# aleju/face-generator

Hardware: NVIDIA H100
Metric: 32x32 GAN train images/sec (1 D-iter + 1 G-iter per batch, batch 256/GPU) (higher is better)
Workload: dtype f32

## Files before the change

face_generator_b200/csrc/capi.cu:

```cuda
#include <algorithm>
#include <cstdarg>
#include <cstdlib>
#include <cstring>

#include "fg_internal.h"
#include "k_conv_tc.h"

static thread_local char g_err[1024] = "";
void fg_set_error(const char* fmt, ...) {
  va_list ap;
  va_start(ap, fmt);
  vsnprintf(g_err, sizeof(g_err), fmt, ap);
  va_end(ap);
}

#define ENTER(c)                                      \
  do {                                                \
    if (!(c)) {                                       \
      fg_set_error("null fg_ctx");                    \
      return FG_ERR_INVALID;                          \
    }                                                 \
    FG_CUDA(cudaSetDevice((c)->device));              \
  } while (0)

// ... 48 lines not shown
  auto dalloc = [c](auto** p, size_t n) { return fg_dalloc(c, c->allocs, reinterpret_cast<float**>(p), n); };
  FG_TRY(dalloc(&c->lop_sx, 2));
  FG_TRY(dalloc(&c->lop_sy, 2));
  FG_TRY(dalloc(&c->seed_dev, 2 * kMaxIters));
  c->splitk_ws_elems = (size_t)c->sm_count * 4 * 128 * 128;
  FG_TRY(dalloc(&c->splitk_ws, c->splitk_ws_elems));
  c->red_ws_elems = (size_t)4 << 20;
  FG_TRY(dalloc(&c->red_ws, 2 * c->red_ws_elems));
  FG_TRY(dalloc(&c->red_ws_opt, 2 * kOptRedRows));
  FG_TRY(dalloc(&c->red_ticket, 2));
  FG_TRY(dalloc(&c->bwd_claim, 1));
  FG_TRY(dalloc(&c->small_ws, (size_t)kSmallMaxParts * 9 * 4 * 128));
  FG_TRY(dalloc(&c->bn_acc, 4 * 256 * 2));
  FG_TRY(dalloc(&c->bn_slice_acc, 32 * 4 * 256 * 2 + 64));
  FG_TRY(dalloc(&c->bn_parts, B * 3072));
  c->io_dev_elems = std::max<size_t>(B * 1024 * C, B * kMaskPerSample);
  return dalloc(&c->io_dev, c->io_dev_elems);
}
void ctx_free(fg_ctx* c) {
  for (void* p : c->allocs) cudaFree(p);
  c->allocs.clear();
  for (int i = 0; i < 8; ++i)
    if (c->scratch[i]) cudaFree(c->scratch[i]);
}
}

extern "C" {

const char* fg_version(void) { return "fg_b200 0.1 (sm_90a)"; }
const char* fg_last_error(void) { return g_err; }
// ... 44 lines not shown
  if (r != FG_OK) {
    net32_free(c);
    ctx_free(c);
    cudaStreamDestroy(c->stream);
    delete c;
    return r;
  }
  *out = c;
  return FG_OK;
}

int fg_destroy(fg_ctx* c) {
  if (!c) return FG_OK;
  cudaSetDevice(c->device);
  cudaStreamSynchronize(c->stream);
  if (c->comm_stream) {
    cudaStreamSynchronize(c->comm_stream);
    cudaStreamDestroy(c->comm_stream);
    cudaEventDestroy(c->ev_fork);
    cudaEventDestroy(c->ev_join);
  }
  tc_destroy(c);
  net32_free(c);
  ctx_free(c);
  for (auto& kv : c->timers)
    for (auto& pr : kv.second.pending) {
      cudaEventDestroy(pr.first);
      cudaEventDestroy(pr.second);
    }
  if (c->own_stream && c->stream) cudaStreamDestroy(c->stream);
  delete c;
  return FG_OK;
}

int fg_set_stream(fg_ctx* c, void* s) {
  ENTER(c);
// ... 213 lines not shown
```

face_generator_b200/csrc/convl.cu:

```cuda
#include "convl.h"

#include "k_conv_tc.h"
#include "k_misc.h"

int convl_dalloc(ConvLEnv& e, float** p, size_t elems) { return fg_dalloc(e.c, *e.allocs, p, elems); }

int ScalePairs::alloc(fg_ctx* c, std::vector<void*>& allocs, int pairs) {
  n = pairs;
  used = 0;
  return fg_dalloc(c, allocs, &base, 2 * (size_t)pairs);
}
int ScalePairs::take(float** pair) {
  if (used == n) {
    fg_set_error("a block of %d FP16 scale pairs is full", n);
    return FG_ERR_UNSUPPORTED;
  }
  *pair = base + 2 * used++;
  return FG_OK;
}
int ScalePairs::reset(fg_ctx* c) const {
  if (!tc_f16(c)) return FG_OK;
  FG_CUDA(cudaMemset2DAsync(base, 2 * sizeof(float), 0, sizeof(float), n, c->stream));
  return FG_OK;
}
// ... 13 lines not shown
      op.split_ready = false;
      return FG_OK;
    }
    return tc_split(c, x, op.hi, op.lo, n);
  }
  if (op.amax_ready) op.amax_ready = false;
  else FG_TRY(tc_amax(c, x, n, op.s));
  return tc_split_h(c, x, op.hi, op.lo, n, op.s);
}

int convl_alloc(ConvLEnv& e, ConvL& L) {
  const size_t nw = (size_t)L.k * L.k * L.Cout * L.Cin;
  FG_TRY(convl_dalloc(e, &L.Wp, nw));
  FG_TRY(convl_dalloc(e, &L.Wpd, nw));
  if (L.nA) FG_TRY(convl_dalloc(e, &L.bp, L.Cout));
  if (!L.x.s) FG_TRY(convl_dalloc(e, &L.x.s, 2));
  if (!e.dy.s) FG_TRY(convl_dalloc(e, &e.dy.s, 2));
  if (tc_conv_eligible(L.geom_k(e.maxB))) {
    const int K = L.geom_k(e.maxB).Cin;
    const size_t nk = (size_t)L.k * L.k * L.Cout * K, nx = (size_t)e.maxB * L.H * L.H * K;
    FG_TRY(convl_dalloc(e, &L.Wf_hi, nk));
    FG_TRY(convl_dalloc(e, &L.Wf_lo, nk));
    FG_TRY(convl_dalloc(e, &L.x.hi, nx));
    FG_TRY(convl_dalloc(e, &L.x.lo, nx));
    if (L.kpad) {
      FG_TRY(convl_dalloc(e, &L.Wpad, nk));
      FG_TRY(convl_dalloc(e, &L.xpad, nx));
    }
  }
  if (L.need_dgrad && tc_conv_eligible(L.geom_d(e.maxB))) {
    FG_TRY(convl_dalloc(e, &L.Wd_hi, nw));
    FG_TRY(convl_dalloc(e, &L.Wd_lo, nw));
  }
  const int B = e.maxB;
  if (L.pad_out && !(tc_conv_eligible(ConvGeom{B, L.H, L.H, L.Cin, L.pad_out, L.k, 1}) &&
                     tc_conv_eligible(ConvGeom{B, L.H, L.H, L.pad_out, L.Cin, L.k, 1}) && L.Cin % 128 == 0))
    L.pad_out = 0;
  if (L.pad_dy && !(L.x.hi && tc_conv_eligible(ConvGeom{B, L.H, L.H, L.Cin, L.pad_dy, L.k, 1}) && L.Cin % 64 == 0))
    L.pad_dy = 0;
  if (L.pad_out) {
    const size_t nq = (size_t)L.k * L.k * L.pad_out * L.Cin;
    FG_TRY(convl_dalloc(e, &L.Wq_hi, nq));
    FG_TRY(convl_dalloc(e, &L.Wq_lo, nq));
    const size_t nx = (size_t)B * L.H * L.H * L.Cin;
    FG_TRY(convl_dalloc(e, &L.x.hi, nx));
    FG_TRY(convl_dalloc(e, &L.x.lo, nx));
  }
  return FG_OK;
}

int convl_pack(fg_ctx* c, ConvL& L, const float* P) {
  const int KK = L.k * L.k;
  const bool tc_on = c->conv_impl != FG_CONV_SIMT;
  const bool h = tc_on && tc_f16(c) && L.geom_k(1).Cin % 64 == 0 && (L.Cout % 64 == 0 || L.pad_out);
  L.packed_f16 = h;
  if (KK > 1 && tc_on && !L.nA && !L.cA && !L.pad_out && !L.kpad && L.Wf_hi && (L.Wd_hi || !L.need_dgrad) && tc_f(c, L, 1) &&
      (!L.need_dgrad || tc_d(c, L, 1))) {
    if (h) return tc_pack_split_h(c, P + L.w_off, L.Wf_hi, L.Wf_lo, L.Wd_hi, L.Wd_lo, L.Cout, L.Cin, KK);
    return tc_pack_split(c, P + L.w_off, L.Wf_hi, L.Wf_lo, L.Wd_hi, L.Wd_lo, L.Cout, L.Cin, KK);
  }
  FG_TRY(k_pack_weights(c, P + L.w_off, L.Wp, L.need_dgrad ? L.Wpd : nullptr, L.Cout, L.Cin, KK, L.nA, L.nS, L.cA, L.cS));
  if (L.bp) FG_TRY(k_pack_weights(c, P + L.b_off, L.bp, nullptr, L.Cout, 1, 1, L.nA, L.nS, 0, 0));
// ... 107 lines not shown

bool upsl_tc(const fg_ctx* c, const UpsL& U) {
  return c->conv_impl != FG_CONV_SIMT && tc_conv_eligible(U.geom(1)) && U.Cout % 128 == 0 && U.Cin % 64 == 0;
}

int upsl_alloc(ConvLEnv& e, UpsL& U) {
  const size_t nw25 = (size_t)25 * U.Cout * U.Cin, nw36 = (size_t)36 * U.Cout * U.Cin;
  FG_TRY(convl_dalloc(e, &U.Wp, nw25));
  FG_TRY(convl_dalloc(e, &U.Wpd, nw25));
  FG_TRY(convl_dalloc(e, &U.Wf_hi, nw36));
  FG_TRY(convl_dalloc(e, &U.Wf_lo, nw36));
  FG_TRY(convl_dalloc(e, &U.Wd_hi, nw36));
  FG_TRY(convl_dalloc(e, &U.Wd_lo, nw36));
  FG_TRY(convl_dalloc(e, &U.Wx_hi, nw25));
  FG_TRY(convl_dalloc(e, &U.Wx_lo, nw25));
  const size_t nx = (size_t)e.maxB * (U.H / 2) * (U.H / 2) * U.Cin;
  FG_TRY(convl_dalloc(e, &U.x.hi, nx));
  FG_TRY(convl_dalloc(e, &U.x.lo, nx));
  if (!U.x.s) FG_TRY(convl_dalloc(e, &U.x.s, 2));
  return FG_OK;
}

int upsl_pack(fg_ctx* c, UpsL& U, const float* P) {
  const float* W = P + U.w_off;
  if (!upsl_tc(c, U)) return k_pack_weights(c, W, U.Wp, U.Wpd, U.Cout, U.Cin, 25, 0, 0, 0, 0);
  if (tc_f16(c)) FG_TRY(tc_pack_collapsed_h(c, W, U.Wf_hi, U.Wf_lo, U.Wd_hi, U.Wd_lo, U.Cout, U.Cin));
  else FG_TRY(tc_pack_collapsed(c, W, U.Wf_hi, U.Wf_lo, U.Wd_hi, U.Wd_lo, U.Cout, U.Cin));
  if (c->conv_impl == FG_CONV_TC_DENSE) FG_TRY(tc_pack_split(c, W, U.Wx_hi, U.Wx_lo, nullptr, nullptr, U.Cout, U.Cin, 25));
  return FG_OK;
}
// ... 53 lines not shown
```

face_generator_b200/csrc/convl.h:

```cpp
#pragma once
#include <vector>

#include "fg_internal.h"

inline bool tc_f16(const fg_ctx* c) { return c->mma_f16 && c->conv_impl == FG_CONV_TC_COLLAPSED; }

struct AmaxInto {
  fg_ctx* c;
  AmaxInto(fg_ctx* c_, TcOp& op) : AmaxInto(c_, op.s, &op.amax_ready) {}
  AmaxInto(fg_ctx* c_, float* pair, bool* done) : c(c_) {
    if (tc_f16(c)) {
      c->amax_out = reinterpret_cast<unsigned*>(pair);
      c->amax_done = done;
    }
  }
  ~AmaxInto() { c->amax_out = nullptr; }
};

inline unsigned* take_amax(fg_ctx* c) {
  unsigned* p = c->amax_out;
  if (p) *c->amax_done = true;
  return p;
}

int tc_op_split(fg_ctx* c, TcOp& op, const float* x, int64_t n, bool f16);

inline int pack_key(const fg_ctx* c) { return c->conv_impl | (c->mma_f16 << 4); }
int convl_dalloc(ConvLEnv& e, float** p, size_t elems);
int convl_alloc(ConvLEnv& e, ConvL& L);
bool convl_tc_fwd(const fg_ctx* c, const ConvL& L);
bool convl_tc_bwd(const fg_ctx* c, const ConvL& L);
int convl_pack(fg_ctx* c, ConvL& L, const float* P);
int convl_fwd(ConvLEnv& e, ConvL& L, const float* in, const float* P, float* out, int B);
int convl_bwd(ConvLEnv& e, ConvL& L, const float* in, const float* dy, float* G, float* din, int B);

bool upsl_tc(const fg_ctx* c, const UpsL& U);
int upsl_alloc(ConvLEnv& e, UpsL& U);
int upsl_pack(fg_ctx* c, UpsL& U, const float* P);
int upsl_fwd(ConvLEnv& e, UpsL& U, const float* h, const float* P, float* z, int B, int* parts = nullptr);
int upsl_bwd(ConvLEnv& e, UpsL& U, TcOp& dy, const float* h, const float* dz, float* G, float* dh, int B, bool* pooled);

int gen_alloc(ConvLEnv& e, UpsGen& G, const GenDesc& d);
int gen_pack(fg_ctx* c, UpsGen& G, NetPair& p);
int gen_forward(ConvLEnv& e, UpsGen& G, NetPair& p, const float* noise, int B, bool training);
int gen_backward(ConvLEnv& e, UpsGen& G, NetPair& p, const float* dy, float* dnoise);
void gen_debug_rows(const UpsGen& G, std::vector<DebugTensor>& rows);
```

face_generator_b200/csrc/fg_internal.h:

```cpp
#pragma once
#include <cuda_runtime.h>
#include <cstdint>
#include <cstdio>
#include <deque>
#include <functional>
#include <initializer_list>
#include <map>
#include <string>
#include <vector>

#include "fg_b200.h"

void fg_set_error(const char* fmt, ...);

#define FG_CUDA(call)                                                                               \
  do {                                                                                              \
    cudaError_t e__ = (call);                                                                       \
    if (e__ != cudaSuccess) {                                                                       \
      fg_set_error("%s:%d: %s -> %s", __FILE__, __LINE__, #call, cudaGetErrorString(e__));          \
      return FG_ERR_CUDA;                                                                           \
    }                                                                                               \
  } while (0)
#define FG_TRY(call)                  \
  do {                                \
// ... 143 lines not shown
};

struct UpsGen {
  int S = 32, C = 3;
  GLayout gl;
  ConvL GL1, GC3;
  UpsL GU[2];
  ScalePairs pairs;
  float* sdz[2] = {nullptr, nullptr};
  float *noise = nullptr, *z0 = nullptr, *h0 = nullptr, *z1 = nullptr, *h1 = nullptr, *z2 = nullptr, *h2 = nullptr,
        *z3 = nullptr, *y = nullptr;
  float *dz3 = nullptr, *dfull = nullptr, *dz2 = nullptr, *dz1 = nullptr, *dz0 = nullptr;
  float *bn_mean[2] = {nullptr, nullptr}, *bn_istd[2] = {nullptr, nullptr}, *bn_mg = nullptr;
  int B = 0;
  bool train = true, valid = false;
  std::deque<std::string> names;
  const char *t_bn2_finalize = nullptr, *t_bn2_stats = nullptr, *t_bn2_apply = nullptr, *t_bn2_bwd_reduce = nullptr,
             *t_bn2_bwd_apply = nullptr;
};

struct TimerRec {
  double ms = 0;
  int64_t launches = 0;
  std::vector<std::pair<cudaEvent_t, cudaEvent_t>> pending;
};

struct IterStage {
  float* p[8] = {};
  size_t cap[8] = {};
  int reserve(fg_ctx* c, std::vector<void*>& allocs, int k, size_t n);
// ... 33 lines not shown
  float* io_dev = nullptr;
  size_t io_dev_elems = 0;
  float* scratch[8] = {nullptr, nullptr, nullptr, nullptr, nullptr, nullptr, nullptr, nullptr};
  size_t scratch_elems[8] = {0, 0, 0, 0, 0, 0, 0, 0};
  void* nccl_comm = nullptr;
  int world = 1, rank = 0;
  int dp_overlap = 1;
  int reserve_sms = 0;
  int last_conv_kind = 0, last_conv_tile_m = 0, last_conv_tile_n = 0, last_conv_format = 0, last_conv_splits = 0;
  int bwd_merge = 1, bwd_merge_ctas = 0;
  int* bwd_claim = nullptr;
  int use_graph = 1, graph_epoch = 0;
  uint64_t* seed_dev = nullptr;
  cudaStream_t comm_stream = nullptr;
  cudaEvent_t ev_fork = nullptr, ev_join = nullptr;
  bool debug_keep = false;
  cudaEvent_t events[16] = {};
  bool timing = false;
  std::map<std::string, TimerRec> timers;
};

inline void note_conv(fg_ctx* c, int kind, int tile_m, int tile_n, int format, int splits) {
  c->last_conv_kind = kind;
  c->last_conv_tile_m = tile_m;
  c->last_conv_tile_n = tile_n;
  c->last_conv_format = format;
  c->last_conv_splits = splits;
}

struct ScopedTimer {
// ... 134 lines not shown
int step_check(fg_ctx* c, const char* what, int B, int nd, int ng, bool inputs, const fg_dataset* d = nullptr, bool fed = false);
struct StepNets {
  StepNets(fg_ctx* c, NetPair& pair, const fg_hyper* h, int B, float* logit, float* out, float* dlogit, float* masks,
           int64_t mask, bool gate, bool overlap)
      : c(c), pair(&pair), h(h), B(B), logit(logit), out(out), dlogit(dlogit), masks(masks), mask(mask), gate(gate),
        overlap(overlap) {}
  fg_ctx* c;
  NetPair* pair;
  const fg_hyper* h;
  int B;
  float *logit, *out, *dlogit;
  float* masks;
  int64_t mask;
  bool gate;
  bool overlap;
  virtual int g_forward(int j, bool d_iter) = 0;
  virtual int d_input(int j) = 0;
  virtual int draw_masks(int kind, const uint64_t* root) = 0;
  virtual int d_forward(bool on_g) = 0;
  virtual int d_backward(bool want_wgrad, bool want_dx) = 0;
  virtual int g_backward() = 0;
};
int pair_train_step(StepNets& s, int nd, int ng, const float* masksD, const float* masksG, uint64_t seed,
                    std::initializer_list<const void*> inputs, const std::function<int()>* feed, fg_step_stats* stats);
struct DebugTensor;
void pair_keep_rows(const NetPair& p, std::vector<DebugTensor>& ents);

int k_relu_fwd(fg_ctx* c, const float* z, float* h, int64_t n);
int k_relu_bwd(fg_ctx* c, const float* dh, const float* z, float* dz, int64_t n);
int k_tanh_dropout_fwd(fg_ctx* c, const float* z, const float* masks_in, const uint64_t* seed_dev, float p, float* code, float* h,
                       float* flags_out, int64_t n);
int k_tanh_dropout_bwd(fg_ctx* c, const float* dh, const float* masks, float p, const float* code, float* dz, int64_t n);
int k_abs_criterion(fg_ctx* c, bool sigmoid, const float* z, const float* t, float* y, float* dz, int64_t n, float* loss);

bool fg_is_dev(const void* p);
int fg_to_dev(fg_ctx* c, const float* p, size_t n, float* staging, const float** out);
int fg_to_user(fg_ctx* c, float* dst, const float* src_dev, size_t n);
// ... 29 lines not shown
```

face_generator_b200/csrc/gen.cu:

```cuda
#include "convl.h"

GLayout make_g_layout(int C, int side) {
  const int64_t n0 = 128 * (side / 4) * (side / 4);
  GLayout L;
  int64_t o = 0;
  L.L1W = o; o += n0 * kNoiseDim;
  L.L1b = o; o += n0;
  L.a1 = o; o += 1;
  L.C1W = o; o += 256 * 128 * 25;
  L.C1b = o; o += 256;
  L.g1 = o; o += 256;
  L.be1 = o; o += 256;
  L.a2 = o; o += 1;
  L.C2W = o; o += 128 * 256 * 25;
  L.C2b = o; o += 128;
  L.g2 = o; o += 128;
  L.be2 = o; o += 128;
  L.a3 = o; o += 1;
  L.C3W = o; o += (int64_t)C * 128 * 9;
  L.C3b = o; o += C;
  L.total = o;
  return L;
}

int gen_alloc(ConvLEnv& e, UpsGen& G, const GenDesc& d) {
  fg_ctx* c = e.c;
  const int S = d.side, C = c->C;
  G.S = S;
  G.C = C;
  G.gl = make_g_layout(C, S);
  const GLayout& gl = G.gl;
  auto timer = [&](const char* name) {
    G.names.push_back(std::string(d.prefix) + name);
    return G.names.back().c_str();
  };
  FG_TRY(G.pairs.alloc(c, *e.allocs, 8));
  ConvL& L1 = G.GL1;
// ... 20 lines not shown
  for (int i = 0; i < 2; ++i) {
    UpsL& U = G.GU[i];
    U.Cin = ci[i]; U.Cout = co[i]; U.H = hs[i];
    U.w_off = wo[i]; U.b_off = bo[i];
    U.tf = timer(uf[i]); U.td = timer(ud[i]); U.tw = timer(uw[i]);
    U.tb = d.bwd_merge ? timer(ub[i]) : nullptr;
    FG_TRY(G.pairs.take(&U.x.s));
    FG_TRY(G.pairs.take(&G.sdz[i]));
    FG_TRY(upsl_alloc(e, U));
  }
  G.t_bn2_finalize = timer("G.bn2.finalize");
  G.t_bn2_stats = timer("hbm.G.bn2.stats");
  G.t_bn2_apply = timer("hbm.G.bn2.apply");
  G.t_bn2_bwd_reduce = timer("hbm.G.bn2.bwd_reduce");
  G.t_bn2_bwd_apply = timer("hbm.G.bn2.bwd_apply");
  const size_t B = e.maxB, n0 = L1.Cout, n1 = (size_t)256 * (S / 2) * (S / 2), n2 = (size_t)128 * S * S, n3 = (size_t)C * S * S;
  for (auto [p, n] : {std::pair<float**, size_t>{&G.noise, kNoiseDim}, {&G.z0, n0}, {&G.h0, n0}, {&G.z1, n1}, {&G.h1, n1},
                      {&G.z2, n2}, {&G.h2, n2}, {&G.z3, n3}, {&G.y, n3}, {&G.dz3, n3},
                      {&G.dfull, (size_t)256 * S * S},
                      {&G.dz2, n2}, {&G.dz1, n1}, {&G.dz0, n0}})
    FG_TRY(convl_dalloc(e, p, B * n));
  for (int i = 0; i < 2; ++i) {
    FG_TRY(convl_dalloc(e, &G.bn_mean[i], co[i]));
    FG_TRY(convl_dalloc(e, &G.bn_istd[i], co[i]));
  }
  return convl_dalloc(e, &G.bn_mg, 512);
}

int gen_pack(fg_ctx* c, UpsGen& G, NetPair& p) {
  if (p.G_pack == pack_key(c)) return FG_OK;
  FG_TRY(convl_pack(c, G.GL1, p.PG));
  for (int i = 0; i < 2; ++i) FG_TRY(upsl_pack(c, G.GU[i], p.PG));
  FG_TRY(convl_pack(c, G.GC3, p.PG));
  p.G_pack = pack_key(c);
  return FG_OK;
}

namespace {
int bn_stats(fg_ctx* c, UpsGen& G, NetPair& p, int i, const float* z, int B, bool training, int parts, const char* t_finalize,
             const char* t_stats) {
  const int Cc = G.GU[i].Cout;
// ... 3 lines not shown
  if (parts) {
    ScopedTimer tm(c, t_finalize);
    return k_bn_finalize_parts(c, c->bn_parts, parts, 4, G.bn_mean[i], G.bn_istd[i], rm, rv, P, Cc);
  }
  {
    ScopedTimer tm(c, t_stats);
    FG_TRY(k_bn_stats(c, z, c->bn_acc, P, Cc));
  }
  return k_bn_finalize(c, c->bn_acc, G.bn_mean[i], G.bn_istd[i], rm, rv, P, Cc);
}
}

int gen_forward(ConvLEnv& e, UpsGen& G, NetPair& p, const float* noise, int B, bool training) {
  fg_ctx* c = e.c;
  FG_REQUIRE(B >= 1 && B <= e.maxB, "G forward: batch %d out of range [1,%d]", B, e.maxB);
  FG_TRY(gen_pack(c, G, p));
  const GLayout& L = G.gl;
  const float* P = p.PG;
  const int S = G.S;
  if (noise != G.noise)
    FG_CUDA(cudaMemcpyAsync(G.noise, noise, sizeof(float) * B * kNoiseDim, cudaMemcpyDeviceToDevice, c->stream));
  G.B = B;
  G.train = training;
  FG_TRY(G.pairs.reset(c));
  FG_TRY(convl_fwd(e, G.GL1, G.noise, P, G.z0, B));
  {
    AmaxInto am(c, G.GU[0].x);
    FG_TRY(k_prelu_fwd(c, G.z0, P + L.a1, G.h0, (int64_t)B * G.GL1.Cout));
  }
  int parts = training ? 1 : 0;
  FG_TRY(upsl_fwd(e, G.GU[0], G.h0, P, G.z1, B, &parts));
// ... 83 lines not shown
```

face_generator_b200/csrc/netpair.cu:

```cuda
#include <algorithm>
#include <cstdlib>
#include <cstring>

#include "convl.h"
#include "fg_internal.h"

namespace {
struct Half {
  float *P, *g, *tail, *m, *v;
  int64_t n;
};
Half half(const NetPair& p, int net) {
  if (net == FG_NET_D) return Half{p.PD, p.gD, p.tailD, p.mD, p.vD, p.nD};
  return Half{p.PG, p.gG, p.tailG, p.mG, p.vG, p.nG};
}
int* step_count(DeviceStats* s, int net) { return net == FG_NET_D ? &s->t_D : &s->t_G; }
}

int fg_dalloc(fg_ctx* c, std::vector<void*>& allocs, float** p, size_t n) {
  void* q = nullptr;
  FG_CUDA(cudaMalloc(&q, std::max<size_t>(n, 1) * sizeof(float)));
  FG_CUDA(cudaMemsetAsync(q, 0, std::max<size_t>(n, 1) * sizeof(float), c->stream));
  allocs.push_back(q);
  *p = (float*)q;
  return FG_OK;
}

int pair_alloc(fg_ctx* c, std::vector<void*>& allocs, NetPair& p, int64_t nG, int64_t nD, bool bn) {
  p.nG = nG;
  p.nD = nD;
  FG_TRY(fg_dalloc(c, allocs, &p.PG, nG));
  FG_TRY(fg_dalloc(c, allocs, &p.PD, nD));
  FG_TRY(fg_dalloc(c, allocs, &p.gG, nG + kGradTail));
  FG_TRY(fg_dalloc(c, allocs, &p.gD, nD + kGradTail));
  p.tailG = p.gG + nG;
  p.tailD = p.gD + nD;
  FG_TRY(fg_dalloc(c, allocs, &p.mG, nG));
  FG_TRY(fg_dalloc(c, allocs, &p.vG, nG));
  FG_TRY(fg_dalloc(c, allocs, &p.mD, nD));
  FG_TRY(fg_dalloc(c, allocs, &p.vD, nD));
// ... 251 lines not shown
  c->launches += e->launches;
  p.G_pack = p.D_pack = -1;
  return FG_OK;
}

namespace {
int keep_dstep(fg_ctx* c, NetPair& p, int B) {
  for (NetPair::Keep& k : p.keep) {
    if (!k.copy) FG_CUDA(cudaMalloc((void**)&k.copy, sizeof(float) * c->maxB * k.per));
    FG_CUDA(cudaMemcpyAsync(k.copy, k.src, sizeof(float) * B * k.per, cudaMemcpyDeviceToDevice, c->stream));
  }
  p.keep_B = B;
  return FG_OK;
}

int step_body(StepNets& s, int nd, int ng, const float* masksD, const float* masksG, const std::function<int()>* feed) {
  fg_ctx* c = s.c;
  NetPair& p = *s.pair;
  const fg_hyper* h = s.h;
  const int B = s.B, Bh = B / 2;
  const size_t mask = (size_t)B * s.mask;
  const float world = (float)c->world;
  fg_hyper hg = *h;
  if (!s.gate) hg.D_maxAcc = 1e30f;
  if (nd > 1 || ng > 1) FG_TRY(k_seed_roots(c, c->seed_dev, std::max(nd, ng)));
  if (feed) FG_TRY((*feed)());
  const bool overlap = s.overlap && c->world > 1 && c->dp_overlap && !c->timing;
  bool forked = false;
  auto g_forward = [&](int j, bool d_iter) -> int {
    static const int reserve = getenv("FG_DP_RESERVE_SMS") ? atoi(getenv("FG_DP_RESERVE_SMS")) : 0;
    c->reserve_sms = forked ? reserve : 0;
    const int r = s.g_forward(j, d_iter);
    c->reserve_sms = 0;
    FG_TRY(r);
    if (forked) FG_CUDA(cudaStreamWaitEvent(c->stream, c->ev_join, 0));
    forked = false;
    return FG_OK;
  };
  auto masks = [&](const float* given, int j, int kind) -> int {
    if (given)
      FG_CUDA(cudaMemcpyAsync(s.masks, given + j * mask, sizeof(float) * mask, cudaMemcpyDeviceToDevice, c->stream));
    else
      FG_TRY(s.draw_masks(kind, c->seed_dev + j));
    return FG_OK;
  };
  for (int j = 0; j < nd; ++j) {
    FG_TRY(g_forward(j, true));
    FG_TRY(s.d_input(j));
    FG_TRY(masks(masksD, j, 1));
    FG_TRY(pair_zero_grads(c, p, FG_NET_D));
    FG_TRY(s.d_forward(false));
    FG_TRY(k_sigmoid_bce(c, s.logit, s.out, s.dlogit, &p.dstats->loss_D, p.tailD, B, Bh));
    if (c->debug_keep) FG_TRY(keep_dstep(c, p, B));
    FG_TRY(s.d_backward(true, false));
    const bool acc = j > 0;
    if (overlap) {
      if (!c->comm_stream) {
        FG_CUDA(cudaStreamCreateWithFlags(&c->comm_stream, cudaStreamNonBlocking));
        FG_CUDA(cudaEventCreateWithFlags(&c->ev_fork, cudaEventDisableTiming));
        FG_CUDA(cudaEventCreateWithFlags(&c->ev_join, cudaEventDisableTiming));
      }
      FG_CUDA(cudaEventRecord(c->ev_fork, c->stream));
      FG_CUDA(cudaStreamWaitEvent(c->comm_stream, c->ev_fork, 0));
      cudaStream_t compute = c->stream;
      c->stream = c->comm_stream;
      int r = pair_allreduce_grads(c, p, FG_NET_D);
      if (r == FG_OK) r = pair_gate(c, p, FG_NET_D, &hg, B, world, acc);
      if (r == FG_OK) r = pair_optim(c, p, FG_NET_D, h, 1.0f / world);
      if (r == FG_OK && cudaEventRecord(c->ev_join, c->comm_stream) != cudaSuccess) r = FG_ERR_CUDA;
      c->stream = compute;
      FG_TRY(r);
      forked = true;
    } else {
      FG_TRY(pair_allreduce_grads(c, p, FG_NET_D));
      FG_TRY(pair_gate(c, p, FG_NET_D, &hg, B, world, acc));
      FG_TRY(pair_optim(c, p, FG_NET_D, h, 1.0f / world));
    }
  }
  for (int j = 0; j < ng; ++j) {
    FG_TRY(pair_zero_grads(c, p, FG_NET_G));
    FG_TRY(g_forward(j, false));
    FG_TRY(masks(masksG, j, 2));
    FG_TRY(s.d_forward(true));
    FG_TRY(k_sigmoid_bce(c, s.logit, s.out, s.dlogit, &p.dstats->loss_G, p.tailG, B, B));
    FG_TRY(s.d_backward(false, true));
    FG_TRY(s.g_backward());
    FG_TRY(pair_allreduce_grads(c, p, FG_NET_G));
    FG_TRY(pair_gate(c, p, FG_NET_G, &hg, B, world));
    FG_TRY(pair_optim(c, p, FG_NET_G, h, 1.0f / world));
  }
  FG_CUDA(cudaMemcpyAsync(p.hstats, p.dstats, sizeof(DeviceStats), cudaMemcpyDeviceToHost, c->stream));
  return FG_OK;
}
}

int pair_train_step(StepNets& s, int nd, int ng, const float* masksD, const float* masksG, uint64_t seed,
// ... 10 lines not shown
```

face_generator_b200/csrc/ups_gan.cu:

```cuda
#include "ups_gan.h"

namespace {
struct GanStep final : StepNets {
  UpsGan& n;
  GanD& D;
  const float *real, *noiseD, *noiseG;
  GanStep(UpsGan& n, const fg_hyper* h, int B, const float* real, const float* noiseD, const float* noiseG)
      : StepNets(n.c, n.net, h, B, n.D->logit, n.D->out, n.D->dlogit, n.D->masks, n.d.mask, true, n.d.overlap), n(n),
        D(*n.D), real(real), noiseD(noiseD), noiseG(noiseG) {}
  int g_forward(int j, bool d_iter) override {
    const int rows = d_iter ? B / 2 : B;
    return gen_forward(n.env, n.G, n.net, (d_iter ? noiseD : noiseG) + (size_t)j * rows * kNoiseDim, rows, true);
  }
  int d_input(int j) override {
    const int Bh = B / 2, HW = n.G.S * n.G.S;
    const size_t img = (size_t)c->C * HW;
    FG_TRY(k_nchw_to_nhwc(c, real + (size_t)j * Bh * img, D.x, Bh, c->C, HW));
    FG_CUDA(cudaMemcpyAsync(D.x + Bh * img, n.G.y, sizeof(float) * Bh * img, cudaMemcpyDeviceToDevice, c->stream));
    return FG_OK;
  }
  int draw_masks(int kind, const uint64_t* root) override { return D.draw_masks(B, kind, h, root); }
  int d_forward(bool on_g) override { return D.forward(on_g ? n.G.y : D.x, B, true, h); }
  int d_backward(bool want_wgrad, bool want_dx) override { return D.backward(want_wgrad, want_dx); }
  int g_backward() override { return gen_backward(n.env, n.G, n.net, D.dx, nullptr); }
};
}

int gan_alloc(UpsGan& n, fg_ctx* c, const GanDesc& d, std::unique_ptr<GanD> D, float* io) {
  n.c = c;
  n.d = d;
  n.D = std::move(D);
  n.D->n = &n;
  ConvLEnv& e = n.env;
  e.c = c;
  e.maxB = c->maxB;
  e.allocs = &n.allocs;
  FG_TRY(pair_alloc(c, n.allocs, n.net, make_g_layout(c->C, d.g.side).total, n.D->layout(c->C), true));
  FG_TRY(n.D->alloc());
  FG_TRY(gen_alloc(e, n.G, d.g));
  const size_t B = c->maxB, img = B * d.g.side * d.g.side * c->C;
  n.img[0] = io;
  if (!io) FG_TRY(convl_dalloc(e, &n.img[0], img));
  FG_TRY(convl_dalloc(e, &n.img[1], img));
  FG_TRY(convl_dalloc(e, &n.z[0], B * kNoiseDim));
  FG_TRY(convl_dalloc(e, &n.z[1], B * kNoiseDim));
  FG_CUDA(cudaStreamSynchronize(c->stream));
  return FG_OK;
}

void gan_free(UpsGan& n) {
  pair_free(n.net);
  n.D.reset();
  for (void* p : n.allocs) cudaFree(p);
  n.allocs.clear();
// ... 123 lines not shown
```

face_generator_b200/csrc/ups_gan.h:

```cpp
#pragma once
#include <memory>
#include <vector>

#include "convl.h"

struct UpsGan;

struct GanD {
  UpsGan* n = nullptr;
  float *x = nullptr, *logit = nullptr, *out = nullptr, *dlogit = nullptr, *masks = nullptr, *dx = nullptr;
  int B = 0;
  virtual ~GanD() = default;
  virtual int64_t layout(int C) = 0;
  virtual int alloc() = 0;
  virtual int forward(const float* x, int B, bool training, const fg_hyper* h) = 0;
  virtual int backward(bool want_wgrad, bool want_dx) = 0;
  virtual int draw_masks(int B, uint64_t seed, const fg_hyper* h, const uint64_t* root) = 0;
  virtual void debug_rows(std::vector<DebugTensor>& rows) const = 0;
};

struct GanDesc {
  GenDesc g;
  int64_t mask;
  bool overlap;
};

struct UpsGan {
  fg_ctx* c = nullptr;
  GanDesc d{};
  NetPair net;
  UpsGen G;
  std::unique_ptr<GanD> D;
  float *img[2] = {nullptr, nullptr}, *z[2] = {nullptr, nullptr};
  IterStage iter_stage;
  std::vector<void*> allocs;
  ConvLEnv env;
};

int gan_alloc(UpsGan& n, fg_ctx* c, const GanDesc& d, std::unique_ptr<GanD> D, float* io);
void gan_free(UpsGan& n);
int gan_pack_D(UpsGan& n, std::initializer_list<ConvL*> layers);
int gan_train_step_iters(UpsGan& n, const char* what, const fg_hyper* h, int B, int d_iters, int g_iters, const float* real,
                         const float* noise_D, const float* noise_G, const float* masks_D, const float* masks_G, uint64_t seed,
                         fg_step_stats* stats);
int gan_train_step_dataset_iters(UpsGan& n, fg_dataset* d, const char* what, const fg_hyper* h, int B, int d_iters,
                                 int g_iters, uint64_t seed, fg_step_stats* stats);
// ... 6 lines not shown
```

Before: 37270.

## Overlap generator forward for G-iter on side stream with discriminator iteration

Measured after the change: 38570, median of 6. 1.04x the previous value.

```diff
diff --git a/face_generator_b200/csrc/capi.cu b/face_generator_b200/csrc/capi.cu
--- a/face_generator_b200/csrc/capi.cu
+++ b/face_generator_b200/csrc/capi.cu
@@ -86,6 +86,12 @@
   FG_TRY(dalloc(&c->bn_acc, 4 * 256 * 2));
   FG_TRY(dalloc(&c->bn_slice_acc, 32 * 4 * 256 * 2 + 64));
   FG_TRY(dalloc(&c->bn_parts, B * 3072));
+  fg_ctx::Workspaces& s = c->side_ws;
+  FG_TRY(dalloc(&s.red_ws, 2 * c->red_ws_elems));
+  FG_TRY(dalloc(&s.red_ticket, 2));
+  FG_TRY(dalloc(&s.bn_acc, 4 * 256 * 2));
+  FG_TRY(dalloc(&s.bn_slice_acc, 32 * 4 * 256 * 2 + 64));
+  FG_TRY(dalloc(&s.bn_parts, B * 3072));
   c->io_dev_elems = std::max<size_t>(B * 1024 * C, B * kMaskPerSample);
   return dalloc(&c->io_dev, c->io_dev_elems);
 }
@@ -160,12 +166,13 @@
   if (!c) return FG_OK;
   cudaSetDevice(c->device);
   cudaStreamSynchronize(c->stream);
-  if (c->comm_stream) {
-    cudaStreamSynchronize(c->comm_stream);
-    cudaStreamDestroy(c->comm_stream);
-    cudaEventDestroy(c->ev_fork);
-    cudaEventDestroy(c->ev_join);
-  }
+  for (cudaStream_t s : {c->comm_stream, c->side_stream})
+    if (s) {
+      cudaStreamSynchronize(s);
+      cudaStreamDestroy(s);
+    }
+  if (c->ev_fork) cudaEventDestroy(c->ev_fork);
+  if (c->ev_join) cudaEventDestroy(c->ev_join);
   tc_destroy(c);
   net32_free(c);
   ctx_free(c);
diff --git a/face_generator_b200/csrc/convl.cu b/face_generator_b200/csrc/convl.cu
--- a/face_generator_b200/csrc/convl.cu
+++ b/face_generator_b200/csrc/convl.cu
@@ -51,19 +51,13 @@
   FG_TRY(convl_dalloc(e, &L.Wp, nw));
   FG_TRY(convl_dalloc(e, &L.Wpd, nw));
   if (L.nA) FG_TRY(convl_dalloc(e, &L.bp, L.Cout));
-  if (!L.x.s) FG_TRY(convl_dalloc(e, &L.x.s, 2));
   if (!e.dy.s) FG_TRY(convl_dalloc(e, &e.dy.s, 2));
-  if (tc_conv_eligible(L.geom_k(e.maxB))) {
-    const int K = L.geom_k(e.maxB).Cin;
-    const size_t nk = (size_t)L.k * L.k * L.Cout * K, nx = (size_t)e.maxB * L.H * L.H * K;
+  const bool tc = tc_conv_eligible(L.geom_k(e.maxB));
+  if (tc) {
+    const size_t nk = (size_t)L.k * L.k * L.Cout * L.geom_k(e.maxB).Cin;
     FG_TRY(convl_dalloc(e, &L.Wf_hi, nk));
     FG_TRY(convl_dalloc(e, &L.Wf_lo, nk));
-    FG_TRY(convl_dalloc(e, &L.x.hi, nx));
-    FG_TRY(convl_dalloc(e, &L.x.lo, nx));
-    if (L.kpad) {
-      FG_TRY(convl_dalloc(e, &L.Wpad, nk));
-      FG_TRY(convl_dalloc(e, &L.xpad, nx));
-    }
+    if (L.kpad) FG_TRY(convl_dalloc(e, &L.Wpad, nk));
   }
   if (L.need_dgrad && tc_conv_eligible(L.geom_d(e.maxB))) {
     FG_TRY(convl_dalloc(e, &L.Wd_hi, nw));
@@ -73,16 +67,24 @@
   if (L.pad_out && !(tc_conv_eligible(ConvGeom{B, L.H, L.H, L.Cin, L.pad_out, L.k, 1}) &&
                      tc_conv_eligible(ConvGeom{B, L.H, L.H, L.pad_out, L.Cin, L.k, 1}) && L.Cin % 128 == 0))
     L.pad_out = 0;
-  if (L.pad_dy && !(L.x.hi && tc_conv_eligible(ConvGeom{B, L.H, L.H, L.Cin, L.pad_dy, L.k, 1}) && L.Cin % 64 == 0))
+  if (L.pad_dy && !(tc && tc_conv_eligible(ConvGeom{B, L.H, L.H, L.Cin, L.pad_dy, L.k, 1}) && L.Cin % 64 == 0))
     L.pad_dy = 0;
   if (L.pad_out) {
     const size_t nq = (size_t)L.k * L.k * L.pad_out * L.Cin;
     FG_TRY(convl_dalloc(e, &L.Wq_hi, nq));
     FG_TRY(convl_dalloc(e, &L.Wq_lo, nq));
-    const size_t nx = (size_t)B * L.H * L.H * L.Cin;
-    FG_TRY(convl_dalloc(e, &L.x.hi, nx));
-    FG_TRY(convl_dalloc(e, &L.x.lo, nx));
-  }
+  }
+  return convl_alloc_x(e, L);
+}
+
+int convl_alloc_x(ConvLEnv& e, ConvL& L) {
+  if (!L.x.s) FG_TRY(convl_dalloc(e, &L.x.s, 2));
+  const bool tc = tc_conv_eligible(L.geom_k(e.maxB));
+  if (!tc && !L.pad_out) return FG_OK;
+  const size_t nx = (size_t)e.maxB * L.H * L.H * L.geom_k(e.maxB).Cin;
+  FG_TRY(convl_dalloc(e, &L.x.hi, nx));
+  FG_TRY(convl_dalloc(e, &L.x.lo, nx));
+  if (tc && L.kpad) FG_TRY(convl_dalloc(e, &L.xpad, nx));
   return FG_OK;
 }
 
@@ -220,6 +222,10 @@
   FG_TRY(convl_dalloc(e, &U.Wd_lo, nw36));
   FG_TRY(convl_dalloc(e, &U.Wx_hi, nw25));
   FG_TRY(convl_dalloc(e, &U.Wx_lo, nw25));
+  return upsl_alloc_x(e, U);
+}
+
+int upsl_alloc_x(ConvLEnv& e, UpsL& U) {
   const size_t nx = (size_t)e.maxB * (U.H / 2) * (U.H / 2) * U.Cin;
   FG_TRY(convl_dalloc(e, &U.x.hi, nx));
   FG_TRY(convl_dalloc(e, &U.x.lo, nx));
diff --git a/face_generator_b200/csrc/convl.h b/face_generator_b200/csrc/convl.h
--- a/face_generator_b200/csrc/convl.h
+++ b/face_generator_b200/csrc/convl.h
@@ -28,6 +28,7 @@
 inline int pack_key(const fg_ctx* c) { return c->conv_impl | (c->mma_f16 << 4); }
 int convl_dalloc(ConvLEnv& e, float** p, size_t elems);
 int convl_alloc(ConvLEnv& e, ConvL& L);
+int convl_alloc_x(ConvLEnv& e, ConvL& L);
 bool convl_tc_fwd(const fg_ctx* c, const ConvL& L);
 bool convl_tc_bwd(const fg_ctx* c, const ConvL& L);
 int convl_pack(fg_ctx* c, ConvL& L, const float* P);
@@ -36,11 +37,13 @@
 
 bool upsl_tc(const fg_ctx* c, const UpsL& U);
 int upsl_alloc(ConvLEnv& e, UpsL& U);
+int upsl_alloc_x(ConvLEnv& e, UpsL& U);
 int upsl_pack(fg_ctx* c, UpsL& U, const float* P);
 int upsl_fwd(ConvLEnv& e, UpsL& U, const float* h, const float* P, float* z, int B, int* parts = nullptr);
 int upsl_bwd(ConvLEnv& e, UpsL& U, TcOp& dy, const float* h, const float* dz, float* G, float* dh, int B, bool* pooled);
 
 int gen_alloc(ConvLEnv& e, UpsGen& G, const GenDesc& d);
+int gen_alloc_fwd(ConvLEnv& e, UpsGen& F, UpsGen& G);
 int gen_pack(fg_ctx* c, UpsGen& G, NetPair& p);
 int gen_forward(ConvLEnv& e, UpsGen& G, NetPair& p, const float* noise, int B, bool training);
 int gen_backward(ConvLEnv& e, UpsGen& G, NetPair& p, const float* dy, float* dnoise);
diff --git a/face_generator_b200/csrc/fg_internal.h b/face_generator_b200/csrc/fg_internal.h
--- a/face_generator_b200/csrc/fg_internal.h
+++ b/face_generator_b200/csrc/fg_internal.h
@@ -181,6 +181,7 @@
   float *bn_mean[2] = {nullptr, nullptr}, *bn_istd[2] = {nullptr, nullptr}, *bn_mg = nullptr;
   int B = 0;
   bool train = true, valid = false;
+  UpsGen* owner = nullptr;
   std::deque<std::string> names;
   const char *t_bn2_finalize = nullptr, *t_bn2_stats = nullptr, *t_bn2_apply = nullptr, *t_bn2_bwd_reduce = nullptr,
              *t_bn2_bwd_apply = nullptr;
@@ -244,6 +245,13 @@
   uint64_t* seed_dev = nullptr;
   cudaStream_t comm_stream = nullptr;
   cudaEvent_t ev_fork = nullptr, ev_join = nullptr;
+  cudaStream_t side_stream = nullptr;
+  struct Workspaces {
+    double* red_ws = nullptr;
+    unsigned* red_ticket = nullptr;
+    double *bn_acc = nullptr, *bn_slice_acc = nullptr;
+    float* bn_parts = nullptr;
+  } side_ws;
   bool debug_keep = false;
   cudaEvent_t events[16] = {};
   bool timing = false;
@@ -408,6 +416,7 @@
   int64_t mask;
   bool gate;
   bool overlap;
+  virtual bool g_side() const { return false; }
   virtual int g_forward(int j, bool d_iter) = 0;
   virtual int d_input(int j) = 0;
   virtual int draw_masks(int kind, const uint64_t* root) = 0;
@@ -415,6 +424,7 @@
   virtual int d_backward(bool want_wgrad, bool want_dx) = 0;
   virtual int g_backward() = 0;
 };
+void ctx_swap_side(fg_ctx* c);
 int pair_train_step(StepNets& s, int nd, int ng, const float* masksD, const float* masksG, uint64_t seed,
                     std::initializer_list<const void*> inputs, const std::function<int()>* feed, fg_step_stats* stats);
 struct DebugTensor;
diff --git a/face_generator_b200/csrc/gen.cu b/face_generator_b200/csrc/gen.cu
--- a/face_generator_b200/csrc/gen.cu
+++ b/face_generator_b200/csrc/gen.cu
@@ -21,6 +21,22 @@
   L.C3b = o; o += C;
   L.total = o;
   return L;
+}
+
+namespace {
+int alloc_fwd(ConvLEnv& e, UpsGen& G) {
+  const int S = G.S;
+  const size_t B = e.maxB, n0 = G.GL1.Cout, n1 = (size_t)256 * (S / 2) * (S / 2), n2 = (size_t)128 * S * S,
+               n3 = (size_t)G.C * S * S;
+  for (auto [p, n] : {std::pair<float**, size_t>{&G.noise, kNoiseDim}, {&G.z0, n0}, {&G.h0, n0}, {&G.z1, n1}, {&G.h1, n1},
+                      {&G.z2, n2}, {&G.h2, n2}, {&G.z3, n3}, {&G.y, n3}})
+    FG_TRY(convl_dalloc(e, p, B * n));
+  for (int i = 0; i < 2; ++i) {
+    FG_TRY(convl_dalloc(e, &G.bn_mean[i], G.GU[i].Cout));
+    FG_TRY(convl_dalloc(e, &G.bn_istd[i], G.GU[i].Cout));
+  }
+  return FG_OK;
+}
 }
 
 int gen_alloc(ConvLEnv& e, UpsGen& G, const GenDesc& d) {
@@ -71,17 +87,43 @@
   G.t_bn2_apply = timer("hbm.G.bn2.apply");
   G.t_bn2_bwd_reduce = timer("hbm.G.bn2.bwd_reduce");
   G.t_bn2_bwd_apply = timer("hbm.G.bn2.bwd_apply");
+  FG_TRY(alloc_fwd(e, G));
   const size_t B = e.maxB, n0 = L1.Cout, n1 = (size_t)256 * (S / 2) * (S / 2), n2 = (size_t)128 * S * S, n3 = (size_t)C * S * S;
-  for (auto [p, n] : {std::pair<float**, size_t>{&G.noise, kNoiseDim}, {&G.z0, n0}, {&G.h0, n0}, {&G.z1, n1}, {&G.h1, n1},
-                      {&G.z2, n2}, {&G.h2, n2}, {&G.z3, n3}, {&G.y, n3}, {&G.dz3, n3},
+  for (auto [p, n] : {std::pair<float**, size_t>{&G.dz3, n3},
                       {&G.dfull, (size_t)256 * S * S},
                       {&G.dz2, n2}, {&G.dz1, n1}, {&G.dz0, n0}})
     FG_TRY(convl_dalloc(e, p, B * n));
-  for (int i = 0; i < 2; ++i) {
-    FG_TRY(convl_dalloc(e, &G.bn_mean[i], co[i]));
-    FG_TRY(convl_dalloc(e, &G.bn_istd[i], co[i]));
-  }
   return convl_dalloc(e, &G.bn_mg, 512);
+}
+
+int gen_alloc_fwd(ConvLEnv& e, UpsGen& F, UpsGen& G) {
+  F.S = G.S;
+  F.C = G.C;
+  F.gl = G.gl;
+  F.owner = &G;
+  F.GL1 = G.GL1;
+  F.GC3 = G.GC3;
+  F.GU[0] = G.GU[0];
+  F.GU[1] = G.GU[1];
+  F.t_bn2_finalize = G.t_bn2_finalize;
+  F.t_bn2_stats = G.t_bn2_stats;
+  F.t_bn2_apply = G.t_bn2_apply;
+  F.t_bn2_bwd_reduce = G.t_bn2_bwd_reduce;
+  F.t_bn2_bwd_apply = G.t_bn2_bwd_apply;
+  FG_TRY(F.pairs.alloc(e.c, *e.allocs, 4));
+  for (ConvL* L : {&F.GL1, &F.GC3}) {
+    L->x = TcOp{};
+    L->xpad = nullptr;
+    L->sdy = nullptr;
+    FG_TRY(F.pairs.take(&L->x.s));
+    FG_TRY(convl_alloc_x(e, *L));
+  }
+  for (UpsL& U : F.GU) {
+    U.x = TcOp{};
+    FG_TRY(F.pairs.take(&U.x.s));
+    FG_TRY(upsl_alloc_x(e, U));
+  }
+  return alloc_fwd(e, F);
 }
 
 int gen_pack(fg_ctx* c, UpsGen& G, NetPair& p) {
@@ -115,7 +157,13 @@
 int gen_forward(ConvLEnv& e, UpsGen& G, NetPair& p, const float* noise, int B, bool training) {
   fg_ctx* c = e.c;
   FG_REQUIRE(B >= 1 && B <= e.maxB, "G forward: batch %d out of range [1,%d]", B, e.maxB);
-  FG_TRY(gen_pack(c, G, p));
+  if (G.owner) {
+    FG_TRY(gen_pack(c, *G.owner, p));
+    G.GL1.packed_f16 = G.owner->GL1.packed_f16;
+    G.GC3.packed_f16 = G.owner->GC3.packed_f16;
+  } else {
+    FG_TRY(gen_pack(c, G, p));
+  }
   const GLayout& L = G.gl;
   const float* P = p.PG;
   const int S = G.S;
diff --git a/face_generator_b200/csrc/netpair.cu b/face_generator_b200/csrc/netpair.cu
--- a/face_generator_b200/csrc/netpair.cu
+++ b/face_generator_b200/csrc/netpair.cu
@@ -24,6 +24,16 @@
   allocs.push_back(q);
   *p = (float*)q;
   return FG_OK;
+}
+
+void ctx_swap_side(fg_ctx* c) {
+  fg_ctx::Workspaces& s = c->side_ws;
+  std::swap(c->stream, c->side_stream);
+  std::swap(c->red_ws, s.red_ws);
+  std::swap(c->red_ticket, s.red_ticket);
+  std::swap(c->bn_acc, s.bn_acc);
+  std::swap(c->bn_slice_acc, s.bn_slice_acc);
+  std::swap(c->bn_parts, s.bn_parts);
 }
 
 int pair_alloc(fg_ctx* c, std::vector<void*>& allocs, NetPair& p, int64_t nG, int64_t nD, bool bn) {
@@ -305,6 +315,13 @@
   return FG_OK;
 }
 
+int fork_init(fg_ctx* c, cudaStream_t* s) {
+  if (!*s) FG_CUDA(cudaStreamCreateWithFlags(s, cudaStreamNonBlocking));
+  if (!c->ev_fork) FG_CUDA(cudaEventCreateWithFlags(&c->ev_fork, cudaEventDisableTiming));
+  if (!c->ev_join) FG_CUDA(cudaEventCreateWithFlags(&c->ev_join, cudaEventDisableTiming));
+  return FG_OK;
+}
+
 int step_body(StepNets& s, int nd, int ng, const float* masksD, const float* masksG, const std::function<int()>* feed) {
   fg_ctx* c = s.c;
   NetPair& p = *s.pair;
@@ -316,6 +333,20 @@
   if (!s.gate) hg.D_maxAcc = 1e30f;
   if (nd > 1 || ng > 1) FG_TRY(k_seed_roots(c, c->seed_dev, std::max(nd, ng)));
   if (feed) FG_TRY((*feed)());
+  const bool side = s.g_side() && c->world == 1 && !c->timing && !c->debug_keep;
+  auto fork_g = [&]() -> int {
+    FG_TRY(fork_init(c, &c->side_stream));
+    FG_CUDA(cudaEventRecord(c->ev_fork, c->stream));
+    FG_CUDA(cudaStreamWaitEvent(c->side_stream, c->ev_fork, 0));
+    ctx_swap_side(c);
+    c->reserve_sms = c->sm_count / 2;
+    int r = pair_zero_grads(c, p, FG_NET_G);
+    if (r == FG_OK) r = s.g_forward(0, false);
+    c->reserve_sms = 0;
+    if (r == FG_OK && cudaEventRecord(c->ev_join, c->stream) != cudaSuccess) r = FG_ERR_CUDA;
+    ctx_swap_side(c);
+    return r;
+  };
   const bool overlap = s.overlap && c->world > 1 && c->dp_overlap && !c->timing;
   bool forked = false;
   auto g_forward = [&](int j, bool d_iter) -> int {
@@ -337,6 +368,7 @@
   };
   for (int j = 0; j < nd; ++j) {
     FG_TRY(g_forward(j, true));
+    if (side && j == nd - 1) FG_TRY(fork_g());
     FG_TRY(s.d_input(j));
     FG_TRY(masks(masksD, j, 1));
     FG_TRY(pair_zero_grads(c, p, FG_NET_D));
@@ -346,11 +378,7 @@
     FG_TRY(s.d_backward(true, false));
     const bool acc = j > 0;
     if (overlap) {
-      if (!c->comm_stream) {
-        FG_CUDA(cudaStreamCreateWithFlags(&c->comm_stream, cudaStreamNonBlocking));
-        FG_CUDA(cudaEventCreateWithFlags(&c->ev_fork, cudaEventDisableTiming));
-        FG_CUDA(cudaEventCreateWithFlags(&c->ev_join, cudaEventDisableTiming));
-      }
+      FG_TRY(fork_init(c, &c->comm_stream));
       FG_CUDA(cudaEventRecord(c->ev_fork, c->stream));
       FG_CUDA(cudaStreamWaitEvent(c->comm_stream, c->ev_fork, 0));
       cudaStream_t compute = c->stream;
@@ -368,9 +396,12 @@
       FG_TRY(pair_optim(c, p, FG_NET_D, h, 1.0f / world));
     }
   }
+  if (side) FG_CUDA(cudaStreamWaitEvent(c->stream, c->ev_join, 0));
   for (int j = 0; j < ng; ++j) {
-    FG_TRY(pair_zero_grads(c, p, FG_NET_G));
-    FG_TRY(g_forward(j, false));
+    if (!side || j > 0) {
+      FG_TRY(pair_zero_grads(c, p, FG_NET_G));
+      FG_TRY(g_forward(j, false));
+    }
     FG_TRY(masks(masksG, j, 2));
     FG_TRY(s.d_forward(true));
     FG_TRY(k_sigmoid_bce(c, s.logit, s.out, s.dlogit, &p.dstats->loss_G, p.tailG, B, B));
diff --git a/face_generator_b200/csrc/ups_gan.cu b/face_generator_b200/csrc/ups_gan.cu
--- a/face_generator_b200/csrc/ups_gan.cu
+++ b/face_generator_b200/csrc/ups_gan.cu
@@ -8,15 +8,17 @@
   GanStep(UpsGan& n, const fg_hyper* h, int B, const float* real, const float* noiseD, const float* noiseG)
       : StepNets(n.c, n.net, h, B, n.D->logit, n.D->out, n.D->dlogit, n.D->masks, n.d.mask, true, n.d.overlap), n(n),
         D(*n.D), real(real), noiseD(noiseD), noiseG(noiseG) {}
+  bool g_side() const override { return true; }
   int g_forward(int j, bool d_iter) override {
     const int rows = d_iter ? B / 2 : B;
-    return gen_forward(n.env, n.G, n.net, (d_iter ? noiseD : noiseG) + (size_t)j * rows * kNoiseDim, rows, true);
+    return gen_forward(d_iter ? n.env_f : n.env, d_iter ? n.F : n.G, n.net,
+                       (d_iter ? noiseD : noiseG) + (size_t)j * rows * kNoiseDim, rows, true);
   }
   int d_input(int j) override {
     const int Bh = B / 2, HW = n.G.S * n.G.S;
     const size_t img = (size_t)c->C * HW;
     FG_TRY(k_nchw_to_nhwc(c, real + (size_t)j * Bh * img, D.x, Bh, c->C, HW));
-    FG_CUDA(cudaMemcpyAsync(D.x + Bh * img, n.G.y, sizeof(float) * Bh * img, cudaMemcpyDeviceToDevice, c->stream));
+    FG_CUDA(cudaMemcpyAsync(D.x + Bh * img, n.F.y, sizeof(float) * Bh * img, cudaMemcpyDeviceToDevice, c->stream));
     return FG_OK;
   }
   int draw_masks(int kind, const uint64_t* root) override { return D.draw_masks(B, kind, h, root); }
@@ -38,6 +40,10 @@
   FG_TRY(pair_alloc(c, n.allocs, n.net, make_g_layout(c->C, d.g.side).total, n.D->layout(c->C), true));
   FG_TRY(n.D->alloc());
   FG_TRY(gen_alloc(e, n.G, d.g));
+  n.env_f.c = c;
+  n.env_f.maxB = c->maxB / 2;
+  n.env_f.allocs = &n.allocs;
+  FG_TRY(gen_alloc_fwd(n.env_f, n.F, n.G));
   const size_t B = c->maxB, img = B * d.g.side * d.g.side * c->C;
   n.img[0] = io;
   if (!io) FG_TRY(convl_dalloc(e, &n.img[0], img));
diff --git a/face_generator_b200/csrc/ups_gan.h b/face_generator_b200/csrc/ups_gan.h
--- a/face_generator_b200/csrc/ups_gan.h
+++ b/face_generator_b200/csrc/ups_gan.h
@@ -30,6 +30,8 @@
   GanDesc d{};
   NetPair net;
   UpsGen G;
+  UpsGen F;
+  ConvLEnv env_f;
   std::unique_ptr<GanD> D;
   float *img[2] = {nullptr, nullptr}, *z[2] = {nullptr, nullptr};
   IterStage iter_stage;
diff --git a/profiles/step_overlap.py b/profiles/step_overlap.py
--- /dev/null
+++ b/profiles/step_overlap.py
@@ -0,0 +1,138 @@
+import argparse
+import json
+import os
+import subprocess
+import sys
+import tempfile
+
+import numpy as np
+
+ROOT = os.path.dirname(os.path.dirname(os.path.abspath(__file__)))
+sys.path.insert(0, ROOT)
+
+
+def card():
+    try:
+        return subprocess.run(["nvidia-smi", "-i", "0", "--query-gpu=name,power.limit,clocks.max.sm", "--format=csv,noheader"],
+                              capture_output=True, text=True, timeout=30).stdout.strip()
+    except Exception as e:
+        return "nvidia-smi unavailable (%s)" % e
+
+
+def union(iv):
+    tot, cur_s, cur_e = 0.0, None, None
+    for s, e in sorted(iv):
+        if cur_e is None or s > cur_e:
+            if cur_e is not None:
+                tot += cur_e - cur_s
+            cur_s, cur_e = s, e
+        else:
+            cur_e = max(cur_e, e)
+    return tot + (cur_e - cur_s if cur_e is not None else 0.0)
+
+
+def overlap(iv):
+    pts = sorted([(s, 1) for s, _ in iv] + [(e, -1) for _, e in iv])
+    tot, depth, last = 0.0, 0, None
+    for t, d in pts:
+        if depth >= 2:
+            tot += t - last
+        depth += d
+        last = t
+    return tot
+
+
+def summarise(kernels, sms):
+    t0 = min(k["ts"] for k in kernels)
+    iv = [(k["ts"], k["ts"] + k["dur"]) for k in kernels]
+    by_stream = {}
+    for k in kernels:
+        by_stream.setdefault(k["stream"], []).append(k)
+    cross = 0.0
+    if len(by_stream) > 1:
+        cross = overlap(iv) - sum(overlap([(k["ts"], k["ts"] + k["dur"]) for k in ks]) for ks in by_stream.values())
+    gaps = {}
+    for s, ks in by_stream.items():
+        ks = sorted(ks, key=lambda k: k["ts"])
+        span = ks[-1]["ts"] + ks[-1]["dur"] - ks[0]["ts"]
+        gaps[s] = {"kernels": len(ks), "span_us": span,
+                   "gaps_us": span - union([(k["ts"], k["ts"] + k["dur"]) for k in ks])}
+    small = [k for k in kernels if k["ctas"] < sms]
+    return {"kernels": len(kernels), "span_us": max(e for _, e in iv) - t0, "busy_us": union(iv),
+            "overlap_us": overlap(iv), "cross_stream_overlap_us": cross, "streams": gaps,
+            "under_one_wave": {"kernels": len(small), "sum_us": sum(k["dur"] for k in small)}}
+
+
+def main():
+    ap = argparse.ArgumentParser()
+    ap.add_argument("--steps", type=int, default=3)
+    ap.add_argument("--warmup", type=int, default=3)
+    ap.add_argument("--batch", type=int, default=256)
+    ap.add_argument("--lib", default=None, help="the libfg_b200.so to load (default: the tree's)")
+    ap.add_argument("--trace", default=None, help="also keep the Chrome trace here")
+    ap.add_argument("--quiet", action="store_true")
+    a = ap.parse_args()
+    import torch
+    from torch.profiler import ProfilerActivity, profile, record_function
+
+    from face_generator_b200.lib import load_library
+    load_library(a.lib)
+    import face_generator_b200 as fg
+    from face_generator_b200 import layouts as LY
+    from face_generator_b200.lib import NET_D, NET_G
+
+    B, C = a.batch, 3
+    torch.cuda.init()
+    sms = torch.cuda.get_device_properties(0).multi_processor_count
+    print("card: %s  (%d SMs)" % (card(), sms))
+    ctx = fg.Context(0, max_batch=B, channels=C)
+    rng = np.random.default_rng(1)
+    ctx.set_params(NET_G, LY.trained_like_init(LY.G_layout(C), rng))
+    ctx.set_params(NET_D, LY.trained_like_init(LY.D_layout(C), rng, 1.4))
+    rng = np.random.default_rng(100)
+    f = lambda x: np.ascontiguousarray(x, np.float32)
+    host = (f(rng.random((B // 2, C, 32, 32))), f(rng.uniform(-1, 1, (B // 2, 100))), f(rng.uniform(-1, 1, (B, 100))))
+    dev = [ctx.dev_array(x) for x in host]
+    hyper = fg.hyper_default()
+    seed = [0]
+
+    def step():
+        seed[0] += 1
+        ctx.train_step(hyper, B, dev[0], dev[1], dev[2], None, None, seed[0], want_stats=False)
+        ctx.sync()
+
+    for _ in range(a.warmup):
+        step()
+    with profile(activities=[ProfilerActivity.CPU, ProfilerActivity.CUDA]) as prof:
+        for i in range(a.steps):
+            with record_function("step%d" % i):
+                step()
+    path = a.trace or os.path.join(tempfile.mkdtemp(), "step_overlap.json")
+    prof.export_chrome_trace(path)
+    ev = json.load(open(path)).get("traceEvents", [])
+    steps = sorted([e for e in ev if e.get("name", "").startswith("step") and e.get("ph") == "X" and
+                    e.get("cat") == "user_annotation"], key=lambda e: e["ts"])
+    kernels = []
+    for e in ev:
+        if e.get("cat") != "kernel" or e.get("ph") != "X":
+            continue
+        g = e.get("args", {}).get("grid", [1, 1, 1])
+        kernels.append({"ts": float(e["ts"]), "dur": float(e["dur"]), "stream": e.get("args", {}).get("stream", e.get("tid")),
+                        "ctas": int(np.prod(g)), "grid": g, "name": e["name"]})
+    for i, s in enumerate(steps):
+        ks = sorted([k for k in kernels if s["ts"] <= k["ts"] <= s["ts"] + s["dur"]], key=lambda k: k["ts"])
+        if not ks:
+            print("step %d: no kernels recorded" % i)
+            continue
+        t0 = ks[0]["ts"]
+        if not a.quiet:
+            print("step %d kernels: stream  start_us  end_us  grid  name" % i)
+            for k in ks:
+                print("  %6s %9.1f %9.1f  %-14s %s" % (k["stream"], k["ts"] - t0, k["ts"] - t0 + k["dur"],
+                                                      "x".join(map(str, k["grid"])), k["name"][:100]))
+        print("step %d summary: %s" % (i, json.dumps(summarise(ks, sms))))
+    ctx.close()
+
+
+if __name__ == "__main__":
+    main()
```
